# fevzibabaoglu/adaptive-edge-aware-jpeg

Hardware: AMD Instinct MI355X
Metric: megapixels/sec encode (Canny+quadtree+DCT+quant), 4K batch (higher is better)
Workload: dtype f32; 1 GPU; 64 x 3840x2160 float32 RGB per GPU, YCbCr, blocks 4-64, quality 40-80 (BASELINE config 4: 512 4K images / 8 GPUs); images_per_gpu=64, height=2160, width=3840, color_space=YCbCr, steps_in_flight=4

## Files before the change

adaptive_edge_aware_jpeg_amd/csrc/aej_common.h:

```cpp
#pragma once
#include <hip/hip_runtime.h>
#include <stdint.h>

namespace aej {

constexpr int kMaxSizes = 8;
constexpr int kClaheTiles = 4;
constexpr int kHystTile = 64;
constexpr int kBlurTW = 64, kBlurTH = 32;
constexpr int kQtChunk = 256;

struct Geom {
    int B;
    int nl;
    int H, W;
    int h[3], w[3];
    int rh[3], rw[3];
    long long poff[3];
    long long pstride;
    int tiled;
    int ctw[3], cth[3];
    int wpr[3];
    long long bpoff[3];
    long long bpstride;
};

struct QtGeom {
    int bmin, bmax;
    int cell;
    int root[3];
    int ncell[3];
    int ltot[3];
    long long pyr_off[3];
    long long pyr_stride;
    int nchunk[3];
    long long chunk_off[3];
    long long chunk_stride;
    long long coeff_off[3], coeff_stride;
    long long leaf_off[3], leaf_stride;
    long long state_off[3], state_stride;
    long long coeff_cap[3], leaf_cap[3], state_cap[3];
    int nsizes;
    long long work_off[3][kMaxSizes], work_stride[kMaxSizes];
};
struct Tuning {
    int color_strip = 1;
    int color_strip_rows = 0;
    int color_workgroups = 0;
    int planes_row_major = 0;
    int dct64_kernel = 0;
    int dct_small_workgroups = 0;
    int sobel_lds = 0;
    int dct_multi = 1;
    int sobel_xcd = 1;
};

#define AEJ_ZIGZAG_8X8                                                                                                                      \
    0, 1, 8, 16, 9, 2, 3, 10, 17, 24, 32, 25, 18, 11, 4, 5, 12, 19, 26, 33, 40, 48, 41, 34, 27, 20, 13, 6, 7, 14, 21, 28, 35, 42, 49, 56, 57, \
        50, 43, 36, 29, 22, 15, 23, 30, 37, 44, 51, 58, 59, 52, 45, 38, 31, 39, 46, 53, 60, 61, 54, 47, 55, 62, 63
struct Zigzag8 {
    unsigned char natural[64], position[64];
};
constexpr Zigzag8 zigzag8_make()
{
    Zigzag8 t = { { AEJ_ZIGZAG_8X8 }, {} };
    for (int z = 0; z < 64; z++) t.position[t.natural[z]] = (unsigned char)z;
    return t;
}
constexpr Zigzag8 kZigzag8 = zigzag8_make();
static __constant__ Zigzag8 k_zigzag8 = zigzag8_make();

constexpr int kChunkInts = 4 + kMaxSizes;
constexpr int kMaxPlanes = 3072;

constexpr int kMetricBand = 32;

struct LeafWork {
    unsigned xy;
    int coef;
};
__host__ __device__ __forceinline__ LeafWork pack_work(int x, int y, int coef)
{
    LeafWork w;
    w.xy = (unsigned)x | ((unsigned)y << 16);
    w.coef = coef;
    return w;
}
// ... 49 lines not shown
```

adaptive_edge_aware_jpeg_amd/csrc/aej_ctx.h:

```cpp
#pragma once
#include <math.h>
#include <stdarg.h>
#include <stdio.h>
#include <string.h>

#include <algorithm>
#include <atomic>
#include <mutex>
#include <string>
#include <thread>
#include <vector>

#include "../../include/aej.h"
#include "../../include/aej_testing.h"
#include "aej_common.h"
#include "aej_launch.h"

struct aej_pending;
constexpr int kFlagWords = 16;
constexpr int kMaxDevices = 64;
struct aej_ctx {
    int device = 0;
    hipStream_t stream = nullptr;
    std::string err;
// ... 6 lines not shown
    const int *d_qm[3][aej::kMaxSizes] = {};
    int *d_check = nullptr;
    const float *d_space_w = nullptr, *d_color_w = nullptr;
    float *d_bilateral = nullptr;
    aej_canny_params canny = { 0.10, 0.30, 0.75, 75.0, 75.0, 1 };
    int *h_flag = nullptr;
    long long last_hyst_queued = 0;
    bool capturing = false;
    long long n_encode_calls = 0;
    int graph_mode = 0;
    hipStream_t gstream = nullptr;
    hipEvent_t gevent = nullptr;
    struct GraphEntry {
        const void *rgb; void *coeffs, *leaves, *states, *counts, *dct, *ws;
        int batch, H, W, in_u8;
        hipGraphExec_t exec;
        unsigned long long last_use;
    };
    std::vector<GraphEntry> graphs;
    unsigned long long graph_clock = 0, n_graph_launches = 0, n_graph_captures = 0;
    int sub_mode = 0;
    int hw_queues = 4;
    int fail_after = -1;
    static constexpr int kMaxSub = 8;
    int dct_crowded = 0;
    hipStream_t sub_stream[kMaxSub] = {};
    hipEvent_t sub_color_done[kMaxSub] = {}, sub_in = nullptr;
    int *sub_flag[kMaxSub] = {};
    long long n_split_calls = 0;
    int sub_chain = -1;
    int chain_hook = 0;
    hipEvent_t chain_event = nullptr;
    aej::Tuning tune;
    int jd_subseq_bits = 2048;
    long long jd_sync_rounds = 0;
    struct aej_pending *pending = nullptr;
    bool profiling = false;
    hipEvent_t ev[24] = {};
    int ev_stage[24] = {};
    int n_ev = 0;
    float stage_ms[AEJ_N_STAGES] = {};
};

namespace aej {
inline int fail(aej_ctx *ctx, int code, const char *fmt, ...)
{
    char buf[512];
    va_list ap;
    va_start(ap, fmt);
    vsnprintf(buf, sizeof buf, fmt, ap);
    va_end(ap);
    if (ctx) ctx->err = buf;
    return code;
}
int hip_fail(aej_ctx *ctx, hipError_t e, const char *expr, const char *file, int line);

inline bool is_pow2(int v) { return v > 0 && (v & (v - 1)) == 0; }
inline long long align_up(long long v, long long a) { return (v + a - 1) / a * a; }

struct Carver {
    char *base;
    unsigned long long off = 0;
    explicit Carver(void *p) : base(static_cast<char *>(p)) {}
    template <typename T> T *take(long long n)
    {
        off = (off + 255) & ~255ull;
// ... 45 lines not shown
```

adaptive_edge_aware_jpeg_amd/csrc/aej_launch.h:

```cpp
#pragma once
#include "aej_common.h"

namespace aej {

int launch_color_convert(hipStream_t st, int space, const float *rgb, float *out, long long n);
bool color_planes_can_tile(const Geom &g, int space, bool in_u8, const Tuning &t);
int launch_color_planes(hipStream_t st, int space, const void *rgb, bool in_u8, const Geom &g, const float *mid, const float *scale,
                        float *raw, float *norm, unsigned char *u8, int *tile_hist, const Tuning &t);
struct AreaTabs {
    int mode;
    int isx, isy;
    const int *xoff, *xsi, *yoff, *ysi;
    const float *xal, *yal;
};
int launch_color_planes_generic(hipStream_t st, int space, const void *rgb, bool in_u8, const Geom &g, const float *mid, const float *scale,
                                const AreaTabs &tabs, float *raw, float *norm, unsigned char *u8, int *tile_hist);
void launch_plane_u8(hipStream_t st, const float *plane, const Geom &g, unsigned char *u8, int *tile_hist);

struct CannyBuffers {
    unsigned char *u8a;
    unsigned char *u8b;
    int *tile_hist;
    unsigned char *lut;
    int *blur_hist;
// ... 8 lines not shown
    double low_q = 0.10 * 100, high_q = 0.30 * 100;
    double clip_limit = 0.75;
    int l2 = 1;
    unsigned char *dump_clahe, *dump_gauss;
};
constexpr int kHystCounters = 128;
long long hyst_tiles_per_image(const Geom &g);
int hyst_ring_slots(const Geom &g);
void launch_clahe_pad_hist(hipStream_t st, const Geom &g, const CannyBuffers &cb);
void launch_clahe_lut(hipStream_t st, const Geom &g, const CannyBuffers &cb);
void launch_clahe_blur(hipStream_t st, const Geom &g, const CannyBuffers &cb);
void launch_thresholds(hipStream_t st, const Geom &g, const CannyBuffers &cb);
void launch_sobel_nms(hipStream_t st, const Geom &g, const CannyBuffers &cb, const Tuning &t);
void launch_hysteresis(hipStream_t st, const Geom &g, const CannyBuffers &cb);
void launch_zero(hipStream_t st, void *p16, size_t bytes_multiple_of_16);
void launch_bits_to_edge(hipStream_t st, const Geom &g, const unsigned long long *strong, unsigned char *edge01);
void launch_bits_to_map(hipStream_t st, const Geom &g, const unsigned long long *weak, const unsigned long long *strong, unsigned char *map);

struct QtBuffers {
    unsigned char *pyr;
    const unsigned long long *edge_bits;
    int *chunk_cnt;
    unsigned short *lane_code;
    int *leaves;
    unsigned char *states;
    long long *counts;
    LeafWork *work[kMaxSizes];
    int *work_count;
    long long work_cap[kMaxSizes];
    int *overflow;
};
void launch_qt_cells(hipStream_t st, const Geom &g, const QtGeom &q, const unsigned long long *edge_bits, const QtBuffers &qb);
void launch_pack_edge_bits(hipStream_t st, const Geom &g, const unsigned char *edge, unsigned long long *bits);
void launch_qt_count(hipStream_t st, const Geom &g, const QtGeom &q, const QtBuffers &qb);
void launch_qt_scan(hipStream_t st, const Geom &g, const QtGeom &q, const QtBuffers &qb);
void launch_qt_emit(hipStream_t st, const Geom &g, const QtGeom &q, const QtBuffers &qb);

constexpr int kBigBlocks = 128;
constexpr int kMaxBlock = 1024;
constexpr int big_blocks(int S) { return S <= 256 ? kBigBlocks : S == 512 ? 64 : 32; }
constexpr long long big_scratch_floats_for(int S) { return S >= 256 ? (long long)big_blocks(S) * S * S : 0; }
struct DctArgs {
    const float *norm;
    int *coeffs;
    float *dct_f32;
    const LeafWork *work;
    float *scratch;
    const int *work_count;
    int k;
    int nplanes;
    const float *D;
    const int *zzinv;
    const int *qm[3];
    int crowded = 0;
};
int launch_dct(hipStream_t st, int size, const Geom &g, const QtGeom &q, const DctArgs &a, long long max_items, const Tuning &t);
int launch_dct_multi(hipStream_t st, const Geom &g, const QtGeom &q, const DctArgs *args, const long long *max_items);
void launch_work_from_leaves(hipStream_t st, const int *leaves, long long n, int bmin, int plane, LeafWork *const *work, int *work_count);


struct IdctArgs {
    const int *coeffs;
    float *planes;
    const LeafWork *work;
    float *scratch;
    const int *work_count;
    int k, nplanes;
    const float *D;
    const int *zz, *zzinv;
// ... 360 lines not shown
```

adaptive_edge_aware_jpeg_amd/csrc/api.hip:

```cpp
#include "aej_ctx.h"

using namespace aej;

int aej::hip_fail(aej_ctx *ctx, hipError_t e, const char *expr, const char *file, int line)
{
    return fail(ctx, AEJ_ERR_HIP, "%s failed: %s (%s:%d)", expr, hipGetErrorString(e), file, line);
}

static const int kRatios[7][3][2] = {
    { { 1, 1 }, { 2, 2 }, { 2, 2 } },
    { { 1, 1 }, { 2, 2 }, { 2, 2 } },
    { { 1, 1 }, { 2, 2 }, { 2, 2 } },
    { { 1, 1 }, { 2, 2 }, { 2, 2 } },
    { { 1, 1 }, { 1, 4 }, { 1, 4 } },
    { { 1, 1 }, { 1, 4 }, { 1, 4 } },
    { { 1, 1 }, { 2, 2 }, { 2, 2 } },
};
const double kMid[7][3] = {
    { 0.5000000037252903, 7.450580596923828e-09, 0.0 }, { 0.5, 0.0, 0.0 }, { 0.5, 0.0, 0.0 },
    { 0.4999999, 0.021152213, -0.056563325 }, { 0.07497266, -0.0008235276, 0.023989676 },
    { 0.07498085, 0.02180194, -0.018250957 }, { 0.0087900255, 0.00048353244, -0.0020741792 },
};
const double kScale[7][3] = {
    { 253.99999810755253, 254.000003784895, 254.0 }, { 254.0, 254.0, 254.0 }, { 254.0, 127.0, 127.0 },
// ... 296 lines not shown
    ctx->graph_mode = mode;
    if (mode == 0) drop_graphs(ctx);
    return 0;
}

extern "C" int aej_set_sub_batches(aej_ctx *ctx, int n)
{
    if (!ctx || n < 0 || n > aej_ctx::kMaxSub) return AEJ_ERR_ARG;
    ctx->sub_mode = n;
    return 0;
}

extern "C" int64_t aej_get_split_calls(aej_ctx *ctx) { return ctx ? (int64_t)ctx->n_split_calls : -1; }

extern "C" int aej_set_hw_queues(aej_ctx *ctx, int n)
{
    if (!ctx || n < 1) return AEJ_ERR_ARG;
    ctx->hw_queues = n;
    return 0;
}

namespace {
struct OptionDef { const char *name; int aej::Tuning::*field; int aej_ctx::*ctx_field; long long lo, hi; bool drops_graphs; };
const OptionDef kOptions[] = {
    { "color_strip", &aej::Tuning::color_strip, nullptr, 0, 1, true },
    { "color_strip_rows", &aej::Tuning::color_strip_rows, nullptr, 0, 64, true },
    { "color_workgroups", &aej::Tuning::color_workgroups, nullptr, 0, 1 << 16, true },
    { "planes_row_major", &aej::Tuning::planes_row_major, nullptr, 0, 1, true },
    { "dct64_kernel", &aej::Tuning::dct64_kernel, nullptr, 0, 4, true },
    { "dct_small_workgroups", &aej::Tuning::dct_small_workgroups, nullptr, 0, 1 << 16, true },
    { "sobel_lds", &aej::Tuning::sobel_lds, nullptr, 0, 1, true },
    { "sobel_xcd", &aej::Tuning::sobel_xcd, nullptr, 0, 1, true },
    { "dct_multi", &aej::Tuning::dct_multi, nullptr, 0, 1, true },
    { "sub_chain", nullptr, &aej_ctx::sub_chain, -1, 3, false },
    { "jpegdec_subseq_bits", nullptr, &aej_ctx::jd_subseq_bits, 32, 1 << 20, false },
};
const OptionDef *find_option(const char *name)
{
    if (!name) return nullptr;
    for (const OptionDef &o : kOptions) if (!strcmp(o.name, name)) return &o;
    return nullptr;
}
}

extern "C" int aej_set_option(aej_ctx *ctx, const char *name, int64_t value)
{
    AEJ_TRY(enter(ctx, __func__));
    const OptionDef *o = find_option(name);
    if (!o) return fail(ctx, AEJ_ERR_ARG, "aej_set_option: unknown option '%s'", name ? name : "(null)");
    if (value < o->lo || value > o->hi || (o->field == &aej::Tuning::dct64_kernel && value != 0 && value != 1 && value != 4))
        return fail(ctx, AEJ_ERR_ARG, "aej_set_option: %s = %lld outside its range [%lld, %lld]", name, (long long)value, o->lo, o->hi);
    if (o->field) ctx->tune.*(o->field) = (int)value;
    else ctx->*(o->ctx_field) = (int)value;
    if (o->drops_graphs) drop_graphs(ctx);
    return 0;
}

extern "C" int aej_get_option(aej_ctx *ctx, const char *name, int64_t *value_host)
{
    if (!ctx || !value_host) return AEJ_ERR_ARG;
    const OptionDef *o = find_option(name);
    if (!o) return fail(ctx, AEJ_ERR_ARG, "aej_get_option: unknown option '%s'", name ? name : "(null)");
    *value_host = o->field ? ctx->tune.*(o->field) : ctx->*(o->ctx_field);
    return 0;
}

// ... 48 lines not shown
```

adaptive_edge_aware_jpeg_amd/csrc/api_encode.hip:

```cpp
#include "aej_ctx.h"

using namespace aej;

static void mark(aej_ctx *ctx, int stage)
{
    if (!ctx->profiling || ctx->n_ev >= 24) return;
    if (!ctx->ev[ctx->n_ev] && hipEventCreate(&ctx->ev[ctx->n_ev]) != hipSuccess) return;
    ctx->ev_stage[ctx->n_ev] = stage;
    (void)hipEventRecord(ctx->ev[ctx->n_ev], ctx->stream);
    ctx->n_ev++;
}

static int injected_failure(aej_ctx *ctx, int stage)
{
    if (ctx->fail_after != stage) return 0;
    ctx->fail_after = -1;
    ctx->err = std::string("injected failure after stage ") + aej_stage_name(stage);
    return AEJ_ERR_STATE;
}

static void collect_marks(aej_ctx *ctx)
{
    for (int i = 0; i < AEJ_N_STAGES; i++) ctx->stage_ms[i] = 0.f;
    for (int i = 1; i < ctx->n_ev; i++) {
// ... 103 lines not shown
{
    hipStream_t st = ctx->stream;
    launch_clahe_pad_hist(st, g, w.cb);
    launch_clahe_lut(st, g, w.cb);
    mark(ctx, AEJ_STAGE_CLAHE_LUT);
    auto publish = [&]() {
        std::lock_guard<std::mutex> lock(g_chain_mutex);
        if (hipEventRecord(ctx->chain_event, st) == hipSuccess) g_last_color_done[ctx->device] = ctx->chain_event;
    };
    launch_clahe_blur(st, g, w.cb);
    mark(ctx, AEJ_STAGE_CLAHE_BLUR);
    if (ctx->chain_hook == 2) publish();
    launch_thresholds(st, g, w.cb);
    mark(ctx, AEJ_STAGE_THRESHOLDS);
    launch_sobel_nms(st, g, w.cb, ctx->tune);
    mark(ctx, AEJ_STAGE_SOBEL_NMS);
    if (ctx->chain_hook == 3) publish();
    launch_hysteresis(st, g, w.cb);
    mark(ctx, AEJ_STAGE_HYSTERESIS);
    AEJ_HIP_CHECK(hipGetLastError());
    return 0;
}

static int clear_canny_ws(aej_ctx *ctx, const CannyWs &w)
{
    if (ctx->capturing) launch_zero(ctx->stream, w.zero_begin, (size_t)(w.zero_end - w.zero_begin));
    else AEJ_HIP_CHECK(hipMemsetAsync(w.zero_begin, 0, (size_t)(w.zero_end - w.zero_begin), ctx->stream));
    return 0;
}

static int run_quadtree(aej_ctx *ctx, const Geom &g, const QtGeom &q, QtWs &w, const unsigned long long *edge_bits)
{
    hipStream_t st = ctx->stream;
    if (ctx->capturing) launch_zero(st, w.zero_begin, (size_t)(w.zero_end - w.zero_begin));
    else AEJ_HIP_CHECK(hipMemsetAsync(w.zero_begin, 0, (size_t)(w.zero_end - w.zero_begin), st));
    w.qb.edge_bits = edge_bits;
    launch_qt_cells(st, g, q, edge_bits, w.qb);
    launch_qt_count(st, g, q, w.qb);
    launch_qt_scan(st, g, q, w.qb);
    launch_qt_emit(st, g, q, w.qb);
    AEJ_HIP_CHECK(hipGetLastError());
    return 0;
}

static void area_tab(int ssize, int dsize, double scale, std::vector<int> &off, std::vector<int> &si, std::vector<float> &alpha)
{
    off.assign((size_t)dsize + 1, 0); si.clear(); alpha.clear();
    for (int dx = 0; dx < dsize; dx++) {
        double fsx1 = dx * scale, fsx2 = fsx1 + scale;
        double cell = scale < ssize - fsx1 ? scale : ssize - fsx1;
        int sx1 = (int)ceil(fsx1), sx2 = (int)floor(fsx2);
        if (sx2 > ssize - 1) sx2 = ssize - 1;
        if (sx1 > sx2) sx1 = sx2;
        off[dx] = (int)si.size();
        if (sx1 - fsx1 > 1e-3) { si.push_back(sx1 - 1); alpha.push_back((float)((sx1 - fsx1) / cell)); }
        for (int sx = sx1; sx < sx2; sx++) { si.push_back(sx); alpha.push_back((float)(1.0 / cell)); }
        if (fsx2 - sx2 > 1e-3) {
            double a = fsx2 - sx2;
            if (a > 1.) a = 1.;
            if (a > cell) a = cell;
            si.push_back(sx2); alpha.push_back((float)(a / cell));
        }
    }
    off[dsize] = (int)si.size();
}

static long long area_tab_ints(const Geom &g)
{
    return 2LL * (g.w[1] + 1 + g.h[1] + 1) + 2LL * (g.W + 2 * g.w[1] + 2) + 2LL * (g.H + 2 * g.h[1] + 2) + 64;
}

static bool planes_fast_ok(const Geom &g)
{
// ... 644 lines not shown
```

adaptive_edge_aware_jpeg_amd/csrc/quadtree.hip:

```cpp
#include "aej_common.h"
#include "aej_launch.h"

namespace aej {

__device__ __forceinline__ unsigned compact1by1(unsigned v)
{
    v &= 0x55555555u;
    v = (v | (v >> 1)) & 0x33333333u;
    v = (v | (v >> 2)) & 0x0F0F0F0Fu;
    v = (v | (v >> 4)) & 0x00FF00FFu;
    v = (v | (v >> 8)) & 0x0000FFFFu;
    return v;
}
__device__ __forceinline__ void morton_decode(unsigned m, int &x, int &y) { x = (int)compact1by1(m); y = (int)compact1by1(m >> 1); }

__device__ __forceinline__ long long lvl_off(int ncell, int lv)
{
    long long o = 0;
    for (int j = 0; j < lv; j++) { long long s = ncell >> j; o += s * s; }
    return o;
}

struct ChunkEdges {
    unsigned e0;
    bool e1, e2, e3, e4;
};

__device__ __forceinline__ ChunkEdges chunk_edges(const Geom &g, const QtGeom &q, int l, int b, const unsigned long long *__restrict__ edge_bits,
                                                  unsigned chunk, int lane)
{
    const int ncell = q.ncell[l], cell = q.cell;
    const int w = g.w[l], h = g.h[l], wpr = g.wpr[l];
    int ccx, ccy, lx, ly;
    morton_decode(chunk, ccx, ccy);
// ... 394 lines not shown
    unsigned char *st = qb.states + (long long)b * q.state_stride + q.state_off[l];
    int *leaves = qb.leaves + ((long long)b * q.leaf_stride + q.leaf_off[l]) * 4;
#pragma unroll
    for (int i = 0; i < 4; i++) {
        for (int k = 0; k < c[i].nsym; k++) {
            if (sym_pos + k < q.state_cap[l]) st[sym_pos + k] = (unsigned char)((c[i].syms >> (2 * k)) & 3u);
            else *qb.overflow = 1;
        }
        sym_pos += c[i].nsym;
        if (c[i].leaf_lvl >= 0) {
            const int cx = cx0 + (i & 1), cy = cy0 + (i >> 1);
            const int size = q.cell << c[i].leaf_lvl;
            if (leaf_pos < q.leaf_cap[l] && (long long)coef_pos + (long long)size * size <= q.coeff_cap[l]) {
                reinterpret_cast<int4 *>(leaves)[leaf_pos] = make_int4(cx * q.cell, cy * q.cell, size, coef_pos);
                if (qb.work_count) {
                    const int k = c[i].leaf_lvl;
                    long long pos = (long long)coff[4 + k] + (k == 0 ? rank0 : rank_big);
                    long long seg = (long long)b * q.work_stride[k] + q.work_off[l][k];
                    if (seg + pos < qb.work_cap[k])
                        qb.work[k][seg + pos] = pack_work(cx * q.cell, cy * q.cell, coef_pos);
                    else
                        *qb.overflow = 1;
                    if (k == 0) rank0++;
                }
            } else {
                *qb.overflow = 1;
            }
            leaf_pos++;
            coef_pos += size * size;
        }
    }
}

static int chunk_blocks(const Geom &g, const QtGeom &q)
{
    int n = 0;
    for (int l = 0; l < g.nl; l++) n += (q.nchunk[l] + 3) / 4;
    return n;
}

void launch_qt_cells(hipStream_t st, const Geom &g, const QtGeom &q, const unsigned long long *edge_bits, const QtBuffers &qb)
{
    bool need = false;
    for (int l = 0; l < g.nl; l++) if (q.ltot[l] > 4 && (q.cell << 5) <= q.bmax) need = true;
    if (need) hipLaunchKernelGGL(k_qt_upper, dim3(chunk_blocks(g, q), g.B), dim3(256), 0, st, g, q, edge_bits, qb.pyr);
}
void launch_qt_count(hipStream_t st, const Geom &g, const QtGeom &q, const QtBuffers &qb)
{
    hipLaunchKernelGGL(k_qt_count, dim3(chunk_blocks(g, q), g.B), dim3(256), 0, st, g, q, qb.edge_bits, qb.pyr, qb.chunk_cnt, qb.lane_code);
}
void launch_qt_scan(hipStream_t st, const Geom &g, const QtGeom &q, const QtBuffers &qb)
{
    if (g.B <= 4) hipLaunchKernelGGL(k_qt_scan<1024>, dim3(g.nl, g.B), dim3(1024), 0, st, g, q, qb.chunk_cnt, qb.counts, qb.work_count);
    else hipLaunchKernelGGL(k_qt_scan<256>, dim3(g.nl, g.B), dim3(256), 0, st, g, q, qb.chunk_cnt, qb.counts, qb.work_count);
}
void launch_qt_emit(hipStream_t st, const Geom &g, const QtGeom &q, const QtBuffers &qb)
{
    hipLaunchKernelGGL(k_qt_emit, dim3(chunk_blocks(g, q), g.B), dim3(256), 0, st, g, q, qb);
}

}
```

Baseline: 83790 MP/s.

## Process quadtree chunks in per-wave runs over only in-image chunks

Adds new count, scan and emit quadtree kernels for cell size 4. Each wave walks a run of consecutive in-image 64x64 chunks across layers and images, prefetching the next chunk's edge bits while it processes the current one. Padding chunks are handled analytically in the scan, so the workspace memset can be skipped when no upper pyramid is needed. This is meant to cut idle work on out-of-image Morton chunks, per-launch grid overhead, and the memset, at the cost of a large new code path that must reproduce the leaf and state output exactly.

```diff
diff --git a/adaptive_edge_aware_jpeg_amd/csrc/aej_common.h b/adaptive_edge_aware_jpeg_amd/csrc/aej_common.h
--- a/adaptive_edge_aware_jpeg_amd/csrc/aej_common.h
+++ b/adaptive_edge_aware_jpeg_amd/csrc/aej_common.h
@@ -53,6 +53,8 @@
     int sobel_lds = 0;
     int dct_multi = 1;
     int sobel_xcd = 1;
+    int qt_chunks = 1;
+    int qt_chunk_run = 0;
 };
 
 #define AEJ_ZIGZAG_8X8                                                                                                                      \
diff --git a/adaptive_edge_aware_jpeg_amd/csrc/aej_ctx.h b/adaptive_edge_aware_jpeg_amd/csrc/aej_ctx.h
--- a/adaptive_edge_aware_jpeg_amd/csrc/aej_ctx.h
+++ b/adaptive_edge_aware_jpeg_amd/csrc/aej_ctx.h
@@ -62,6 +62,7 @@
     int chain_hook = 0;
     hipEvent_t chain_event = nullptr;
     aej::Tuning tune;
+    int qt_chunk_launches = 0;
     int jd_subseq_bits = 2048;
     long long jd_sync_rounds = 0;
     struct aej_pending *pending = nullptr;
diff --git a/adaptive_edge_aware_jpeg_amd/csrc/aej_launch.h b/adaptive_edge_aware_jpeg_amd/csrc/aej_launch.h
--- a/adaptive_edge_aware_jpeg_amd/csrc/aej_launch.h
+++ b/adaptive_edge_aware_jpeg_amd/csrc/aej_launch.h
@@ -64,9 +64,18 @@
 };
 void launch_qt_cells(hipStream_t st, const Geom &g, const QtGeom &q, const unsigned long long *edge_bits, const QtBuffers &qb);
 void launch_pack_edge_bits(hipStream_t st, const Geom &g, const unsigned char *edge, unsigned long long *bits);
-void launch_qt_count(hipStream_t st, const Geom &g, const QtGeom &q, const QtBuffers &qb);
-void launch_qt_scan(hipStream_t st, const Geom &g, const QtGeom &q, const QtBuffers &qb);
-void launch_qt_emit(hipStream_t st, const Geom &g, const QtGeom &q, const QtBuffers &qb);
+struct QtRuns {
+    int ncx0, ncx1, ncx2;
+    int ncy0, ncy1, ncy2;
+    int nin0, nin1, nin2;
+    int per_image, total;
+    int run;
+};
+bool qt_chunk_runs(const Geom &g, const QtGeom &q, const Tuning &t, QtRuns &r);
+bool qt_needs_upper(const Geom &g, const QtGeom &q);
+void launch_qt_count(hipStream_t st, const Geom &g, const QtGeom &q, const QtBuffers &qb, const QtRuns *runs);
+void launch_qt_scan(hipStream_t st, const Geom &g, const QtGeom &q, const QtBuffers &qb, const QtRuns *runs);
+void launch_qt_emit(hipStream_t st, const Geom &g, const QtGeom &q, const QtBuffers &qb, const QtRuns *runs);
 
 constexpr int kBigBlocks = 128;
 constexpr int kMaxBlock = 1024;
diff --git a/adaptive_edge_aware_jpeg_amd/csrc/api.hip b/adaptive_edge_aware_jpeg_amd/csrc/api.hip
--- a/adaptive_edge_aware_jpeg_amd/csrc/api.hip
+++ b/adaptive_edge_aware_jpeg_amd/csrc/api.hip
@@ -352,6 +352,9 @@
     { "sobel_lds", &aej::Tuning::sobel_lds, nullptr, 0, 1, true },
     { "sobel_xcd", &aej::Tuning::sobel_xcd, nullptr, 0, 1, true },
     { "dct_multi", &aej::Tuning::dct_multi, nullptr, 0, 1, true },
+    { "qt_chunks", &aej::Tuning::qt_chunks, nullptr, 0, 1, true },
+    { "qt_chunk_run", &aej::Tuning::qt_chunk_run, nullptr, 0, 16, true },
+    { "qt_chunk_launches", nullptr, &aej_ctx::qt_chunk_launches, 0, 0x7fffffff, false },
     { "sub_chain", nullptr, &aej_ctx::sub_chain, -1, 3, false },
     { "jpegdec_subseq_bits", nullptr, &aej_ctx::jd_subseq_bits, 32, 1 << 20, false },
 };
diff --git a/adaptive_edge_aware_jpeg_amd/csrc/api_encode.hip b/adaptive_edge_aware_jpeg_amd/csrc/api_encode.hip
--- a/adaptive_edge_aware_jpeg_amd/csrc/api_encode.hip
+++ b/adaptive_edge_aware_jpeg_amd/csrc/api_encode.hip
@@ -159,13 +159,16 @@
 static int run_quadtree(aej_ctx *ctx, const Geom &g, const QtGeom &q, QtWs &w, const unsigned long long *edge_bits)
 {
     hipStream_t st = ctx->stream;
+    QtRuns runs_of_call;
+    const QtRuns *runs = qt_chunk_runs(g, q, ctx->tune, runs_of_call) ? &runs_of_call : nullptr;
     if (ctx->capturing) launch_zero(st, w.zero_begin, (size_t)(w.zero_end - w.zero_begin));
-    else AEJ_HIP_CHECK(hipMemsetAsync(w.zero_begin, 0, (size_t)(w.zero_end - w.zero_begin), st));
+    else if (qt_needs_upper(g, q) || !runs) AEJ_HIP_CHECK(hipMemsetAsync(w.zero_begin, 0, (size_t)(w.zero_end - w.zero_begin), st));
     w.qb.edge_bits = edge_bits;
     launch_qt_cells(st, g, q, edge_bits, w.qb);
-    launch_qt_count(st, g, q, w.qb);
-    launch_qt_scan(st, g, q, w.qb);
-    launch_qt_emit(st, g, q, w.qb);
+    launch_qt_count(st, g, q, w.qb, runs);
+    launch_qt_scan(st, g, q, w.qb, runs);
+    launch_qt_emit(st, g, q, w.qb, runs);
+    if (runs) ctx->qt_chunk_launches++;
     AEJ_HIP_CHECK(hipGetLastError());
     return 0;
 }
diff --git a/adaptive_edge_aware_jpeg_amd/csrc/quadtree.hip b/adaptive_edge_aware_jpeg_amd/csrc/quadtree.hip
--- a/adaptive_edge_aware_jpeg_amd/csrc/quadtree.hip
+++ b/adaptive_edge_aware_jpeg_amd/csrc/quadtree.hip
@@ -1,5 +1,7 @@
 #include "aej_common.h"
 #include "aej_launch.h"
+#include <algorithm>
+#include <string.h>
 
 namespace aej {
 
@@ -460,6 +462,438 @@
     }
 }
 
+constexpr int kQtCell = 4;
+
+template <class T> __device__ __forceinline__ T sel3(T a, T b, T c, int l) { return l == 0 ? a : l == 1 ? b : c; }
+
+__device__ __forceinline__ unsigned part1by1(unsigned v)
+{
+    v &= 0x0000FFFFu;
+    v = (v | (v << 8)) & 0x00FF00FFu;
+    v = (v | (v << 4)) & 0x0F0F0F0Fu;
+    v = (v | (v << 2)) & 0x33333333u;
+    v = (v | (v << 1)) & 0x55555555u;
+    return v;
+}
+
+struct QtLayer {
+    int w, h, wpr, ncw, nch;
+    int ncx, nin, ltot, ncell;
+    long long bp_base, pyr_base, rec_base;
+};
+__device__ __forceinline__ QtLayer select_layer(const Geom &g, const QtGeom &q, const QtRuns &R, int l, int b)
+{
+    QtLayer L;
+    L.w = g.w[l]; L.h = g.h[l]; L.wpr = g.wpr[l];
+    L.ncw = (L.w + kQtCell - 1) / kQtCell; L.nch = (L.h + kQtCell - 1) / kQtCell;
+    L.ncx = sel3(R.ncx0, R.ncx1, R.ncx2, l); L.nin = sel3(R.nin0, R.nin1, R.nin2, l);
+    L.ltot = q.ltot[l]; L.ncell = q.ncell[l];
+    L.bp_base = (long long)b * g.bpstride + g.bpoff[l];
+    L.pyr_base = (long long)b * q.pyr_stride + q.pyr_off[l];
+    L.rec_base = (long long)b * q.chunk_stride + q.chunk_off[l];
+    return L;
+}
+
+struct QtCursor { int b, l, col, row, r; };
+__device__ __forceinline__ QtCursor cursor_at(const QtRuns &R, int gi)
+{
+    QtCursor c;
+    c.b = gi / R.per_image;
+    int r = gi - c.b * R.per_image;
+    c.l = 0;
+    if (r >= R.nin0) { r -= R.nin0; c.l = 1; if (r >= R.nin1) { r -= R.nin1; c.l = 2; } }
+    const int ncx = sel3(R.ncx0, R.ncx1, R.ncx2, c.l);
+    c.r = r; c.row = r / ncx; c.col = r - c.row * ncx;
+    return c;
+}
+__device__ __forceinline__ bool cursor_next(QtCursor &c, const QtLayer &L, int nl)
+{
+    c.r++; c.col++;
+    if (c.col == L.ncx) { c.col = 0; c.row++; }
+    if (c.r < L.nin) return false;
+    c.r = c.col = c.row = 0;
+    if (++c.l == nl) { c.l = 0; c.b++; }
+    return true;
+}
+
+__device__ __forceinline__ bool pyr_at(const unsigned char *__restrict__ pyr, int ncell, int lv, int cx, int cy)
+{
+    const int side = ncell >> lv;
+    return pyr[lvl_off(ncell, lv) + (long long)(cy >> lv) * side + (cx >> lv)] != 0;
+}
+
+struct QtUpper { int n_up, up_leaf; bool x4; };
+__device__ __forceinline__ QtUpper upper_walk(const QtGeom &q, const QtLayer &L, const unsigned char *__restrict__ pyr, unsigned chunk, int col, int row)
+{
+    QtUpper u;
+    u.n_up = 0; u.up_leaf = -1; u.x4 = false;
+    const int a = chunk == 0 ? L.ltot : min(4 + ((__ffs((int)chunk) - 1) >> 1), L.ltot);
+    if ((kQtCell << 5) > q.bmax) {
+        u.n_up = a - 4; u.x4 = true;
+        return u;
+    }
+    const int cx = col * 16, cy = row * 16;
+    if (a < L.ltot) {
+        const int psize = kQtCell << (a + 1);
+        if (!(psize > q.bmax || pyr_at(pyr, L.ncell, a + 1, cx, cy))) return u;
+    }
+    for (int lv = a; lv >= 5; lv--) {
+        if ((kQtCell << lv) > q.bmax || pyr_at(pyr, L.ncell, lv, cx, cy)) u.n_up++;
+        else { u.up_leaf = lv; return u; }
+    }
+    u.x4 = true;
+    return u;
+}
+
+__device__ __forceinline__ unsigned long long spread4(unsigned long long m) { m &= 0x1111111111111111ull; return (m << 4) - m; }
+__device__ __forceinline__ unsigned long long spread16(unsigned long long m) { m &= 0x0001000100010001ull; return (m << 16) - m; }
+__device__ __forceinline__ unsigned long long any4(unsigned long long m) { return spread4(m | (m >> 1) | (m >> 2) | (m >> 3)); }
+__device__ __forceinline__ unsigned long long any16(unsigned long long m) { return spread16(m | (m >> 4) | (m >> 8) | (m >> 12)); }
+__device__ __forceinline__ bool bit_of(unsigned long long m, int lane) { return (m >> lane) & 1ull; }
+
+__global__ __launch_bounds__(256) void k_qt_count_chunks(Geom g, QtGeom q, QtRuns R, const unsigned long long *__restrict__ edge_bits,
+                                                         const unsigned char *__restrict__ pyr_all, int4 *__restrict__ chunk_rec,
+                                                         unsigned short *__restrict__ lane_code, int *__restrict__ overflow)
+{
+    if (blockIdx.x == 0 && threadIdx.x == 0) *overflow = 0;
+    const int wave = __builtin_amdgcn_readfirstlane((int)(blockIdx.x * 4 + (threadIdx.x >> 6)));
+    const int lane = threadIdx.x & 63;
+    const int gi0 = wave * R.run, gi1 = min(gi0 + R.run, R.total);
+    if (gi0 >= gi1) return;
+    int lx, ly;
+    morton_decode((unsigned)lane, lx, ly);
+    QtCursor c = cursor_at(R, gi0);
+    QtLayer L = select_layer(g, q, R, c.l, c.b);
+    struct Res { long long rec_i; unsigned code; int4 r0, r1, r2; };
+    auto put = [&](const Res &r) __attribute__((always_inline)) {
+        lane_code[r.rec_i * 64 + lane] = (unsigned short)r.code;
+        chunk_rec[3 * r.rec_i] = r.r0; chunk_rec[3 * r.rec_i + 1] = r.r1; chunk_rec[3 * r.rec_i + 2] = r.r2;
+    };
+    auto request = [&](unsigned long long (&raw)[8]) __attribute__((always_inline)) {
+        const unsigned long long *tile = edge_bits + L.bp_base + (unsigned)(c.row * L.wpr + c.col) * 64u + 8 * ly;
+#pragma unroll
+        for (int r = 0; r < 8; r++) raw[r] = tile[r];
+    };
+    const unsigned long long big1 = (kQtCell << 1) > q.bmax ? ~0ull : 0ull, big2 = (kQtCell << 2) > q.bmax ? ~0ull : 0ull, big3 = (kQtCell << 3) > q.bmax ? ~0ull : 0ull;
+    auto work = [&](unsigned long long (&raw)[8]) __attribute__((always_inline)) {
+        const unsigned chunk = part1by1((unsigned)c.col) | (part1by1((unsigned)c.row) << 1);
+        const long long rec_i = L.rec_base + chunk;
+        if (c.row * 64 + 64 > L.h) {
+            const int rows = L.h - c.row * 64 - 8 * ly;
+#pragma unroll
+            for (int r = 0; r < 8; r++) raw[r] = r < rows ? raw[r] : 0ull;
+        }
+        unsigned long long top = raw[0] | raw[1] | raw[2] | raw[3], bot = raw[4] | raw[5] | raw[6] | raw[7];
+        const unsigned t8 = (unsigned)(top >> (8 * lx)) & 0xFFu, b8 = (unsigned)(bot >> (8 * lx)) & 0xFFu;
+        const unsigned e0 = ((t8 & 0x0Fu) ? 1u : 0u) | ((t8 & 0xF0u) ? 2u : 0u) | ((b8 & 0x0Fu) ? 4u : 0u) | ((b8 & 0xF0u) ? 8u : 0u);
+        const unsigned long long E1 = __ballot(e0 != 0);
+        const QtUpper u = upper_walk(q, L, pyr_all + L.pyr_base, chunk, c.col, c.row);
+        const bool top_exists = u.x4 || u.up_leaf >= 0 || u.n_up > 0;
+        const bool S4 = (kQtCell << 4) > q.bmax || E1 != 0;
+        int nsym = u.n_up + (u.up_leaf >= 0 ? 1 : 0) + (u.x4 ? 1 : 0);
+        int lf[5] = { 0, 0, 0, 0, 0 };
+        unsigned code = 0;
+        if (!(u.x4 && S4)) {
+            lf[4] = u.x4 ? 1 : 0;
+            if (lane == 0 && top_exists) code = 1u | ((unsigned)u.n_up << 2);
+        } else {
+            const int cx0 = c.col * 16 + 2 * lx, cy0 = c.row * 16 + 2 * ly;
+            const bool interior = c.col * 16 + 16 <= L.ncw && c.row * 16 + 16 <= L.nch;
+            unsigned long long inx0 = ~0ull, inx1 = ~0ull, iny0 = ~0ull, iny1 = ~0ull;
+            if (!interior) {
+                inx0 = __ballot(cx0 < L.ncw); inx1 = __ballot(cx0 + 1 < L.ncw);
+                iny0 = __ballot(cy0 < L.nch); iny1 = __ballot(cy0 + 1 < L.nch);
+            }
+            const unsigned long long IN1 = inx0 & iny0, IN2 = spread4(IN1), IN3 = spread16(IN1);
+            const unsigned long long E2 = any4(E1), E3 = any16(E2);
+            const unsigned long long S1 = E1 | big1, S2 = E2 | big2, S3 = E3 | big3;
+            const unsigned long long X3 = ~0ull, X2 = X3 & IN3 & S3, X1 = X2 & IN2 & S2, X0 = X1 & IN1 & S1;
+            const unsigned long long F2 = 0x1111111111111111ull, F3 = 0x0001000100010001ull;
+            lf[3] = __popcll(X3 & IN3 & ~S3 & F3);
+            lf[2] = __popcll(X2 & IN2 & ~S2 & F2);
+            lf[1] = __popcll(X1 & IN1 & ~S1);
+            lf[0] = __popcll(X0 & inx0 & iny0) + __popcll(X0 & inx1 & iny0) + __popcll(X0 & inx0 & iny1) + __popcll(X0 & inx1 & iny1);
+            nsym += 4 + __popcll(X2 & F2) + __popcll(X1) + 4 * __popcll(X0);
+            const bool s1 = bit_of(S1, lane), s2 = bit_of(S2, lane), s3 = bit_of(S3, lane), in1 = bit_of(IN1, lane);
+            const int c1 = s1 ? 1 : 0, c2 = s2 ? 1 + c1 : 0, c3 = s3 ? 1 + c2 : 0;
+            const int a = 1 + ((__ffs(lane | 64) - 1) >> 1);
+            bool ex = a == 1 ? bit_of(X1, lane) : a == 2 ? bit_of(X2, lane) : true;
+            int kk = a == 1 ? c1 : a == 2 ? c2 : c3;
+            if (lane == 0) { ex = true; kk = u.n_up + 1 + c3; }
+            code = !ex ? 0u : !in1 ? 3u : (1u | ((unsigned)kk << 2));
+            if (bit_of(X0, lane)) {
+                const bool x1 = cx0 + 1 < L.ncw, y1 = cy0 + 1 < L.nch;
+                code |= (x1 ? 1u : 3u) << 6 | (y1 ? 1u : 3u) << 8 | (x1 && y1 ? 1u : 3u) << 10;
+            }
+        }
+        Res res;
+        res.rec_i = rec_i; res.code = code;
+        const int nleaf = lf[0] + lf[1] + lf[2] + lf[3] + lf[4] + (u.up_leaf >= 0 ? 1 : 0);
+        int ncoef = 0;
+#pragma unroll
+        for (int k = 0; k < 5; k++) ncoef += lf[k] * (kQtCell << k) * (kQtCell << k);
+        if (u.up_leaf >= 0) ncoef += (kQtCell << u.up_leaf) * (kQtCell << u.up_leaf);
+        static_assert(kMaxSizes == 8, "a chunk record holds eight per-size counts");
+        res.r0 = make_int4(nsym, nleaf, ncoef, 0);
+        res.r1 = make_int4(lf[0], lf[1], lf[2], lf[3]);
+        res.r2 = make_int4(lf[4], u.up_leaf == 5 ? 1 : 0, u.up_leaf == 6 ? 1 : 0, u.up_leaf == 7 ? 1 : 0);
+        return res;
+    };
+    unsigned long long raw[8];
+    request(raw);
+    Res res = work(raw);
+    for (int gi = gi0 + 1; gi < gi1; gi++) {
+        if (cursor_next(c, L, g.nl)) L = select_layer(g, q, R, c.l, c.b);
+        request(raw);
+        put(res);
+        res = work(raw);
+    }
+    put(res);
+}
+
+template <int kScanThreads>
+__global__ __launch_bounds__(kScanThreads) void k_qt_scan_chunks(Geom g, QtGeom q, QtRuns R, int4 *__restrict__ rec_all, const unsigned char *__restrict__ pyr_all,
+                                                                 unsigned char *__restrict__ states, long long *__restrict__ counts,
+                                                                 int *__restrict__ work_count, int *__restrict__ overflow)
+{
+    constexpr int NQ = 3 + kMaxSizes;
+    __shared__ int s_w[NQ][kScanThreads / 64];
+    __shared__ int carry[NQ];
+    const int tid = threadIdx.x, l = blockIdx.x, b = blockIdx.y;
+    const int lane = tid & 63, wv = tid >> 6;
+    int4 *rec = rec_all + ((long long)b * q.chunk_stride + q.chunk_off[l]) * 3;
+    const unsigned char *pyr = pyr_all + (long long)b * q.pyr_stride + q.pyr_off[l];
+    unsigned char *st = states + (long long)b * q.state_stride + q.state_off[l];
+    const int n = q.nchunk[l], ncell = q.ncell[l], ncx = sel3(R.ncx0, R.ncx1, R.ncx2, l), ncy = sel3(R.ncy0, R.ncy1, R.ncy2, l);
+    const long long state_cap = q.state_cap[l];
+    const int nq = 3 + q.nsizes;
+    if (tid < NQ) carry[tid] = 0;
+    __syncthreads();
+    static_assert(kChunkInts == 12 && NQ == 11, "a chunk record is three int4: (nsym, nleaf, ncoef, pad), leaves per size 0..3, 4..7");
+    for (int start = 0; start < n; start += kScanThreads) {
+        const int i = start + tid;
+        int4 r0 = make_int4(0, 0, 0, 0), r1 = r0, r2 = r0;
+        bool inside = false;
+        if (i < n) {
+            int ccx, ccy;
+            morton_decode((unsigned)i, ccx, ccy);
+            inside = ccx < ncx && ccy < ncy;
+            if (inside) { r0 = rec[3 * i]; r1 = rec[3 * i + 1]; r2 = rec[3 * i + 2]; }
+            else {
+                const int p = 5 + ((__ffs(i) - 1) >> 1), sh = p - 4;
+                const int pcx = (ccx >> sh) << sh, pcy = (ccy >> sh) << sh;
+                if (pcx < ncx && pcy < ncy && ((kQtCell << p) > q.bmax || pyr_at(pyr, ncell, p, pcx * 16, pcy * 16))) r0.x = 1;
+            }
+        }
+        int v[NQ] = { r0.x, r0.y, r0.z, r1.x, r1.y, r1.z, r1.w, r2.x, r2.y, r2.z, r2.w }, inc[NQ];
+#pragma unroll
+        for (int c = 0; c < NQ; c++) {
+            if (c >= nq) v[c] = 0;
+            inc[c] = wave_incl_scan(v[c], lane);
+            if (lane == 63) s_w[c][wv] = inc[c];
+        }
+        __syncthreads();
+        int o[NQ];
+#pragma unroll
+        for (int c = 0; c < NQ; c++) {
+            int p = carry[c];
+            for (int k = 0; k < wv; k++) p += s_w[c][k];
+            o[c] = p + inc[c] - v[c];
+        }
+        if (inside) {
+            rec[3 * i] = make_int4(o[0], o[1], o[2], r0.w);
+            rec[3 * i + 1] = make_int4(o[3], o[4], o[5], o[6]);
+            rec[3 * i + 2] = make_int4(o[7], o[8], o[9], o[10]);
+        } else if (r0.x) {
+            if (o[0] < state_cap) st[o[0]] = (unsigned char)2;
+            else *overflow = 1;
+        }
+        __syncthreads();
+        if (tid < NQ) {
+            int t = 0;
+            for (int k = 0; k < kScanThreads / 64; k++) t += s_w[tid][k];
+            carry[tid] += t;
+        }
+        __syncthreads();
+    }
+    if (tid == 0) {
+        long long *o = counts + ((long long)b * 3 + l) * 4;
+        o[0] = carry[2];
+        o[1] = carry[1];
+        o[2] = carry[0];
+        o[3] = q.root[l];
+    }
+    if (work_count && tid < kMaxSizes) work_count[((long long)b * 3 + l) * kMaxSizes + tid] = tid < q.nsizes ? carry[3 + tid] : 0;
+}
+
+constexpr int kQtMaxRun = 16;
+constexpr int kQtStageStates = 512;
+
+__device__ __forceinline__ void wave_lds_sync()
+{
+    __builtin_amdgcn_fence(__ATOMIC_RELEASE, "wavefront");
+    __builtin_amdgcn_wave_barrier();
+    __builtin_amdgcn_fence(__ATOMIC_ACQUIRE, "wavefront");
+}
+
+__global__ __launch_bounds__(256) void k_qt_emit_chunks(Geom g, QtGeom q, QtRuns R, QtBuffers qb, const int *__restrict__ chunk_rec,
+                                                        const unsigned short *__restrict__ lane_code)
+{
+    __shared__ int4 s_leaf_all[4][kQtChunk];
+    __shared__ unsigned char s_state_all[4][kQtStageStates];
+    const int wv = threadIdx.x >> 6;
+    int4 *s_leaf = s_leaf_all[wv];
+    unsigned char *s_state = s_state_all[wv];
+    const int wave = __builtin_amdgcn_readfirstlane((int)(blockIdx.x * 4 + wv));
+    const int lane = threadIdx.x & 63;
+    const int gi0 = wave * R.run, n = min(R.run, R.total - gi0);
+    if (n <= 0) return;
+    int lx, ly;
+    morton_decode((unsigned)lane, lx, ly);
+    const QtCursor c0 = cursor_at(R, gi0);
+    const QtLayer L0 = select_layer(g, q, R, c0.l, c0.b);
+
+    unsigned pk[kQtMaxRun / 2];
+    long long my_rec = 0;
+    {
+        QtCursor c = c0;
+        QtLayer L = L0;
+        unsigned code[kQtMaxRun];
+#pragma unroll
+        for (int i = 0; i < kQtMaxRun; i++) {
+            const unsigned chunk = part1by1((unsigned)c.col) | (part1by1((unsigned)c.row) << 1);
+            const long long rec_i = L.rec_base + chunk;
+            code[i] = lane_code[rec_i * 64 + lane];
+            if ((lane >> 2) == i) my_rec = rec_i;
+            if (i + 1 < n && cursor_next(c, L, g.nl)) L = select_layer(g, q, R, c.l, c.b);
+        }
+#pragma unroll
+        for (int j = 0; j < kQtMaxRun / 2; j++) pk[j] = code[2 * j] | (code[2 * j + 1] << 16);
+    }
+    const int *my = chunk_rec + my_rec * kChunkInts + (lane & 3);
+    const int v_pos = my[0], v_szlo = my[4], v_szhi = my[8];
+
+    struct Out { long long state_cap, leaf_cap, coeff_cap, seg0; unsigned char *st; int4 *leaves; };
+    auto select_out = [&](int l, int b) {
+        Out o;
+        o.state_cap = q.state_cap[l]; o.leaf_cap = q.leaf_cap[l]; o.coeff_cap = q.coeff_cap[l];
+        o.st = qb.states + (long long)b * q.state_stride + q.state_off[l];
+        o.leaves = reinterpret_cast<int4 *>(qb.leaves) + ((long long)b * q.leaf_stride + q.leaf_off[l]);
+        o.seg0 = (long long)b * q.work_stride[0] + q.work_off[l][0];
+        return o;
+    };
+    QtCursor c = c0;
+    QtLayer L = L0;
+    Out O = select_out(c.l, c.b);
+    const bool lists = qb.work_count != nullptr;
+    const unsigned long long lt_mask = (1ull << lane) - 1ull;
+    for (int i = 0; i < n; i++) {
+        const unsigned code = pk[0] & 0xFFFFu;
+#pragma unroll
+        for (int j = 0; j < kQtMaxRun / 2 - 1; j++) pk[j] = (pk[j] >> 16) | (pk[j + 1] << 16);
+        pk[kQtMaxRun / 2 - 1] >>= 16;
+        const unsigned long long originators = __ballot(code != 0);
+        if (originators != 0) {
+            const unsigned chunk = part1by1((unsigned)c.col) | (part1by1((unsigned)c.row) << 1);
+            const int sym_base = __builtin_amdgcn_readlane(v_pos, 4 * i), leaf_base = __builtin_amdgcn_readlane(v_pos, 4 * i + 1);
+            const int coef_base = __builtin_amdgcn_readlane(v_pos, 4 * i + 2), szoff0 = __builtin_amdgcn_readlane(v_szlo, 4 * i);
+            const long long state_cap = O.state_cap, leaf_cap = O.leaf_cap, coeff_cap = O.coeff_cap;
+            unsigned char *st = O.st;
+            int4 *leaves = O.leaves;
+            const long long seg0 = O.seg0 + szoff0;
+            const unsigned t = code & 3u;
+            const int k0 = (int)((code >> 2) & 15u);
+            const unsigned ci[3] = { (code >> 6) & 3u, (code >> 8) & 3u, (code >> 10) & 3u };
+            const int a_chunk = chunk == 0 ? L.ltot : min(4 + ((__ffs((int)chunk) - 1) >> 1), L.ltot);
+            const int a = lane == 0 ? a_chunk : 1 + ((__ffs(lane) - 1) >> 1);
+            const int lvl0 = t == 1u ? a - k0 : -1;
+            const int size0 = lvl0 >= 0 ? kQtCell << lvl0 : 0;
+            const int nsym0 = t == 0u ? 0 : t == 3u ? 1 : k0 + (t == 1u ? 1 : 0);
+            const int x0 = (c.col * 16 + 2 * lx) * kQtCell, y0 = (c.row * 16 + 2 * ly) * kQtCell;
+            bool fit0 = false;
+            int coef0 = coef_base;
+            if (originators == 1ull && __ballot((code >> 6) != 0u) == 0ull) {
+                if (lane == 0) {
+                    for (int k = 0; k < nsym0; k++) {
+                        if (sym_base + k < state_cap) st[sym_base + k] = (unsigned char)(t == 3u ? 2 : k < k0 ? 1 : 0); else *qb.overflow = 1;
+                    }
+                    if (lvl0 >= 0) {
+                        fit0 = leaf_base < leaf_cap && (long long)coef_base + (long long)size0 * size0 <= coeff_cap;
+                        if (fit0) leaves[leaf_base] = make_int4(x0, y0, size0, coef_base); else *qb.overflow = 1;
+                        if (fit0 && lists && lvl0 == 0) {
+                            if (seg0 < qb.work_cap[0]) qb.work[0][seg0] = pack_work(x0, y0, coef_base); else *qb.overflow = 1;
+                        }
+                    }
+                }
+            } else {
+                const int nl13 = (ci[0] == 1u ? 1 : 0) + (ci[1] == 1u ? 1 : 0) + (ci[2] == 1u ? 1 : 0);
+                const int nsym = nsym0 + (ci[0] ? 1 : 0) + (ci[1] ? 1 : 0) + (ci[2] ? 1 : 0);
+                const int nleaf = (lvl0 >= 0 ? 1 : 0) + nl13;
+                const int ncoef = size0 * size0 + nl13 * kQtCell * kQtCell;
+                const int pk2 = nsym | nleaf << 10;
+                const int inc2 = wave_incl_scan(pk2, lane), inc_c = wave_incl_scan(ncoef, lane);
+                const int tot2 = __builtin_amdgcn_readlane(inc2, 63);
+                const int tsym = tot2 & 1023, tleaf = (tot2 >> 10) & 1023;
+                int lsym = (inc2 - pk2) & 1023, lleaf = ((inc2 - pk2) >> 10) & 1023, coef_pos = coef_base + inc_c - ncoef;
+                coef0 = coef_pos;
+                for (int k = 0; k < nsym0; k++) s_state[lsym + k] = (unsigned char)(t == 3u ? 2 : k < k0 ? 1 : 0);
+                lsym += nsym0;
+                if (lvl0 >= 0) {
+                    fit0 = leaf_base + lleaf < leaf_cap && (long long)coef_pos + (long long)size0 * size0 <= coeff_cap;
+                    s_leaf[lleaf++] = make_int4(x0, y0, size0, coef_pos);
+                    coef_pos += size0 * size0;
+                }
+#pragma unroll
+                for (int j = 0; j < 3; j++)
+                    if (ci[j]) {
+                        s_state[lsym++] = (unsigned char)(ci[j] == 1u ? 0 : ci[j] == 2u ? 1 : 2);
+                        if (ci[j] == 1u) {
+                            s_leaf[lleaf++] = make_int4(x0 + ((j + 1) & 1) * kQtCell, y0 + ((j + 1) >> 1) * kQtCell, kQtCell, coef_pos);
+                            coef_pos += kQtCell * kQtCell;
+                        }
+                    }
+                wave_lds_sync();
+                for (int j = lane; j < tsym; j += 64) {
+                    if (sym_base + j < state_cap) st[sym_base + j] = s_state[j]; else *qb.overflow = 1;
+                }
+                int run0 = 0;
+                for (int j0 = 0; j0 < tleaf; j0 += 64) {
+                    const int j = j0 + lane;
+                    const bool valid = j < tleaf;
+                    int4 e = make_int4(0, 0, 0, 0);
+                    if (valid) e = s_leaf[j];
+                    const bool fit = valid && leaf_base + j < leaf_cap && (long long)e.w + (long long)e.z * e.z <= coeff_cap;
+                    if (fit) leaves[leaf_base + j] = e;
+                    else if (valid) *qb.overflow = 1;
+                    if (lists) {
+                        const bool is0 = valid && e.z == kQtCell;
+                        const unsigned long long m0 = __ballot(is0);
+                        if (is0 && fit) {
+                            const long long pos = seg0 + run0 + __popcll(m0 & lt_mask);
+                            if (pos < qb.work_cap[0]) qb.work[0][pos] = pack_work(e.x, e.y, e.w); else *qb.overflow = 1;
+                        }
+                        run0 += __popcll(m0);
+                    }
+                }
+                wave_lds_sync();
+            }
+            if (lists && __ballot(lvl0 > 0) != 0) {
+                for (int k = 1; k < q.nsizes; k++) {
+                    const unsigned long long mk = __ballot(lvl0 == k);
+                    if (mk == 0) continue;
+                    const int szoff = __builtin_amdgcn_readlane(k < 4 ? v_szlo : v_szhi, 4 * i + (k & 3));
+                    const long long seg = (long long)c.b * q.work_stride[k] + q.work_off[c.l][k] + szoff;
+                    if (lvl0 == k && fit0) {
+                        const long long pos = seg + __popcll(mk & lt_mask);
+                        if (pos < qb.work_cap[k]) qb.work[k][pos] = pack_work(x0, y0, coef0); else *qb.overflow = 1;
+                    }
+                }
+            }
+        }
+        if (i + 1 < n && cursor_next(c, L, g.nl)) { L = select_layer(g, q, R, c.l, c.b); O = select_out(c.l, c.b); }
+    }
+}
+
 static int chunk_blocks(const Geom &g, const QtGeom &q)
 {
     int n = 0;
@@ -467,24 +901,62 @@
     return n;
 }
 
+bool qt_needs_upper(const Geom &g, const QtGeom &q)
+{
+    for (int l = 0; l < g.nl; l++) if (q.ltot[l] > 4 && (q.cell << 5) <= q.bmax) return true;
+    return false;
+}
+
+bool qt_chunk_runs(const Geom &g, const QtGeom &q, const Tuning &t, QtRuns &R)
+{
+    memset(&R, 0, sizeof R);
+    if (!t.qt_chunks || q.cell != kQtCell || q.bmin != kQtCell || g.nl < 1 || g.nl > 3) return false;
+    long long per_image = 0;
+    int ncx[3] = { 0, 0, 0 }, ncy[3] = { 0, 0, 0 };
+    for (int l = 0; l < g.nl; l++) {
+        if (q.ltot[l] < 4) return false;
+        ncx[l] = (g.w[l] + 63) / 64; ncy[l] = (g.h[l] + 63) / 64;
+        per_image += (long long)ncx[l] * ncy[l];
+    }
+    R.ncx0 = ncx[0]; R.ncx1 = ncx[1]; R.ncx2 = ncx[2];
+    R.ncy0 = ncy[0]; R.ncy1 = ncy[1]; R.ncy2 = ncy[2];
+    R.nin0 = ncx[0] * ncy[0]; R.nin1 = ncx[1] * ncy[1]; R.nin2 = ncx[2] * ncy[2];
+    const long long total = per_image * g.B;
+    if (total >= (1ll << 30)) return false;
+    R.per_image = (int)per_image; R.total = (int)total;
+    R.run = (int)std::min<long long>(kQtMaxRun, std::max<long long>(1, (total + 4095) / 4096));
+    if (t.qt_chunk_run > 0) R.run = std::min(t.qt_chunk_run, kQtMaxRun);
+    return true;
+}
+static unsigned run_blocks(const QtRuns &R) { return (unsigned)(((R.total + R.run - 1) / R.run + 3) / 4); }
+
 void launch_qt_cells(hipStream_t st, const Geom &g, const QtGeom &q, const unsigned long long *edge_bits, const QtBuffers &qb)
 {
-    bool need = false;
-    for (int l = 0; l < g.nl; l++) if (q.ltot[l] > 4 && (q.cell << 5) <= q.bmax) need = true;
-    if (need) hipLaunchKernelGGL(k_qt_upper, dim3(chunk_blocks(g, q), g.B), dim3(256), 0, st, g, q, edge_bits, qb.pyr);
-}
-void launch_qt_count(hipStream_t st, const Geom &g, const QtGeom &q, const QtBuffers &qb)
-{
-    hipLaunchKernelGGL(k_qt_count, dim3(chunk_blocks(g, q), g.B), dim3(256), 0, st, g, q, qb.edge_bits, qb.pyr, qb.chunk_cnt, qb.lane_code);
-}
-void launch_qt_scan(hipStream_t st, const Geom &g, const QtGeom &q, const QtBuffers &qb)
-{
+    if (qt_needs_upper(g, q)) hipLaunchKernelGGL(k_qt_upper, dim3(chunk_blocks(g, q), g.B), dim3(256), 0, st, g, q, edge_bits, qb.pyr);
+}
+void launch_qt_count(hipStream_t st, const Geom &g, const QtGeom &q, const QtBuffers &qb, const QtRuns *runs)
+{
+    if (runs)
+        hipLaunchKernelGGL(k_qt_count_chunks, dim3(run_blocks(*runs)), dim3(256), 0, st, g, q, *runs, qb.edge_bits, qb.pyr, reinterpret_cast<int4 *>(qb.chunk_cnt),
+                           qb.lane_code, qb.overflow);
+    else
+        hipLaunchKernelGGL(k_qt_count, dim3(chunk_blocks(g, q), g.B), dim3(256), 0, st, g, q, qb.edge_bits, qb.pyr, qb.chunk_cnt, qb.lane_code);
+}
+void launch_qt_scan(hipStream_t st, const Geom &g, const QtGeom &q, const QtBuffers &qb, const QtRuns *runs)
+{
+    if (runs) {
+        int4 *rec = reinterpret_cast<int4 *>(qb.chunk_cnt);
+        if (g.B <= 4) hipLaunchKernelGGL(k_qt_scan_chunks<1024>, dim3(g.nl, g.B), dim3(1024), 0, st, g, q, *runs, rec, qb.pyr, qb.states, qb.counts, qb.work_count, qb.overflow);
+        else hipLaunchKernelGGL(k_qt_scan_chunks<256>, dim3(g.nl, g.B), dim3(256), 0, st, g, q, *runs, rec, qb.pyr, qb.states, qb.counts, qb.work_count, qb.overflow);
+        return;
+    }
     if (g.B <= 4) hipLaunchKernelGGL(k_qt_scan<1024>, dim3(g.nl, g.B), dim3(1024), 0, st, g, q, qb.chunk_cnt, qb.counts, qb.work_count);
     else hipLaunchKernelGGL(k_qt_scan<256>, dim3(g.nl, g.B), dim3(256), 0, st, g, q, qb.chunk_cnt, qb.counts, qb.work_count);
 }
-void launch_qt_emit(hipStream_t st, const Geom &g, const QtGeom &q, const QtBuffers &qb)
-{
-    hipLaunchKernelGGL(k_qt_emit, dim3(chunk_blocks(g, q), g.B), dim3(256), 0, st, g, q, qb);
-}
-
-}
+void launch_qt_emit(hipStream_t st, const Geom &g, const QtGeom &q, const QtBuffers &qb, const QtRuns *runs)
+{
+    if (runs) hipLaunchKernelGGL(k_qt_emit_chunks, dim3(run_blocks(*runs)), dim3(256), 0, st, g, q, *runs, qb, qb.chunk_cnt, qb.lane_code);
+    else hipLaunchKernelGGL(k_qt_emit, dim3(chunk_blocks(g, q), g.B), dim3(256), 0, st, g, q, qb);
+}
+
+}
```

After: 86220 MP/s (median of 6 runs). +2.9%, better.
